# maikmerten/hmp3

Measured on AMD Instinct MI355X. Metric: batched stereo 44.1kHz frames/sec (whole node), CBR-128, higher is better.
Workload: dtype f32; 1 GPU; batch=1024 stereo 44.1kHz streams x 256 frames per step per GPU, CBR-128, long blocks only, int16 PCM resident in HBM; streams_per_gpu=1024, parallelism=streams sharded over 1 GPU(s), no collective

## Files before the change

### hmp3_amd/csrc/hx_alloc.hip

```cpp
#include "hx_dev.h"

#ifndef HX_LSF
#define HX_LSF 0
#endif
#ifndef HX_A1
#define HX_A1 0
#endif
#ifndef HX_SLIM
#define HX_SLIM 0
#endif
#if HX_SLIM && HX_A1
#error "the low-footprint layout is built for the second-generation allocator only"
#endif
#define HX_WAVES (HX_SLIM ? 3 : 2)
#define HX_PERSIST HX_SLIM
#define HX_RATE_SPEED (!HX_SLIM)
#define HX_OPAQUE_LANE HX_SLIM
#define HX_SEEK_FORCEINLINE HX_SLIM
#define HX_LUCKY_K (HX_SLIM ? 6 : 12)
#define GMIN_OFFSET 70
#define PART23 4021
#define NB 22

struct AllocPrm {
    unsigned char head[4];
    int remainder, divisor, main_framebytes, sf_bit_max, AveTargetBits;
    int ms_flag, hf_flag, vbr_flag;
    int ivbr_min, ivbr_max, vbr_main_framebytes[16], vbr_pool_target;
    int fbmin, fbmax;
    int initialMNR, test1;
    int nsf[2], nsf2[2], nsf3[2], nbmax[2], nbmax2[2], nbmax3[2];
    float rnBand_l[22];
    int nsfs, nbmax_s;
    struct { int npart; } psyS;
    int nchan, side_bytes;
    int is_flag, dual, npart_l;
    int oflags;
    int run_w;
};

static_assert(sizeof(HxGr) == 96, "the frame loop copies the four HxGr of a frame as 96 words");
struct alignas(16) Outbox {
    HxSegOut seg[2];
    HxGr gr[2][2];
    int scfsi[2], mdb, part;
    unsigned sidew[10];
    unsigned char head[4];
    HxFrameOut frm;
    HxSlot slot;
    int opos, frm_index, slot_index;
    int ring_p0;
    int has_frame;
};

#if HX_SLIM
typedef short ix_t;
typedef short sgs_t;
typedef signed char sfo_t;
typedef short btab_t;
#else
typedef int ix_t;
typedef int sgs_t;
typedef int sfo_t;
typedef int btab_t;
#endif

struct FrameState {
    int padcount; unsigned main_tot, main_sent, mf_tot;
    int main_bytes; unsigned side_p0, side_p1, tot_frames_out, tot_bytes_out; int ave_tot;
    int opos, slot_lo, slot_hi;
    int pad, byte_pool, byte_max, byte_min, bytesout, pk_first;
};

struct alignas(16) AllocLds {
    float xr[2][576];
    float x34[2][576];
    float term[2][576];
#if !HX_SLIM
    int ix[2][576];
    unsigned char signx[2][576];
    alignas(16) HxBandPrep band_next;
#else
    unsigned long long sgnbits[2][9];
    ix_t ixsink;
#endif
    unsigned char band_of_pair[288];
    unsigned short lane_run[64];
    unsigned char band_last[24];
    float look_ix43[256];
#if !HX_SLIM
    float look_gain[128], look_34igain[128];
    int mblog[256];
    float pow34_exp[256];
    int logsub[84];
#else
    float gain4[4], igain16[16];
    unsigned short mblog[256];
    short logsub[84];
#endif
    float pow34_a[16], pow34_b[16], quant_off[32];
    unsigned char huff_len[1408];
    unsigned char sband_of_line[192];
    btab_t nBand_s[16], startBand_s[16], logcbw_s[16];
    unsigned char quada_len[16];
    btab_t nBand[NB], startBand[24], logcbw[NB], taper[NB];
    int NTadjust[2][NB];
    union {
        struct {
            int snr[2][NB], Noise0[2][NB], Noise[2][NB], NT[2][NB];
            int gzero[2][NB], gmin[2][NB], gsf[2][NB], sf[2][NB], active[2][NB];
            int ixmax[2][NB], ix10xmax[2][NB], up[2][NB], lo[2][NB], geval[2][NB], maskmb[2][NB];
            float xsxx[2][NB], x34max[2][NB];
            float gig[2][NB];
            alignas(8) float2 gpair[2][NB];
            int lucky[HX_LUCKY_K][2][13];
            unsigned short llist[HX_LUCKY_K * 26 + 4];
        };
        struct {
            int a_pad[17][2][NB];
            float a_sig[2][NB], a_smask[2][NB], a_mask[2][NB], a_noise[2][NB];
            int a_lastGsf[2][NB];
        };
        struct {
            int s_snr[2][3][16], s_Noise0[2][3][16], s_Noise[2][3][16], s_NT[2][3][16];
            sgs_t s_gzero[2][3][16], s_gmin[2][3][16], s_gsf[2][3][16], s_sf[2][3][16], s_active[2][3][16];
            int s_ixmax[2][3][16], s_geval[3][16], s_tmpn[3][16], s_maskmb[2][3][16];
            float s_xsxx[2][3][16], s_x34max[2][3][16];
            int s_G[2][3], s_GG[2], s_subgain[2][3];
        };
    };
    int G[2], preemp[2], scale[2], huff_bits[2];
    int hs_table[2][4], hs_cbreg[2][3], hs_nbig[2], hs_nquads[2], hs_bits[2];
    int MNR, PoolFraction, call_count;
    int a_calls, a_bitadjust[2];
    float a_running, a_ave, a_alpha;
    int hf_quant, hf_quant_stereo[2], gsf_hf, gsf_hf_stereo[2];
    int sf_save[2][21];
    int scfsi[2];
    int nchan, block_type, maxBits, maxTargetBits, minTargetBits, PoolBits, TargetBits, deltaMNR, activeBands;
    int tmp[8];
    int tmpn[2][NB];
    unsigned int sidew[10];
    HxGr gr[2][2];
    sfo_t sfout[2][2][NB];
    sfo_t sfs[2][3][12];
    AllocPrm P;
    FrameState fs;
    int tabpk[32];
    unsigned long long candpk[19];
    unsigned short r_mf[32];
    int r_off[32];
#if !HX_SLIM
    float dump[64];
#endif
    Outbox ob[2];
    const double *pow43;
    int *big_counter;
    int nstrict;
#if !HX_SLIM
    int nlucky[3];
#endif
    int cur_s;
    alignas(16) int cmdw[4];
    alignas(4) unsigned char gflag[HX_SLIM ? 64 : 256];
#ifdef HX_PROFILE
    unsigned prof[HX_PROF_WORDS];
#endif
};

#if !HX_SLIM
// ... 88 lines not shown
    const unsigned seg = (u >> 19) & 15;
    const int e = (int) ((u >> 23) & 255), k = 3 * (e - 127);
    float ex = ldexpf(L.gain4[k & 3], k >> 2);
    if (e == 0) ex = 0.0f;
    if (e == 255) ex = hx_bits2f(0x7F800000u);
    return (m * L.pow34_b[seg] + L.pow34_a[seg]) * ex;
}
#else
__device__ __forceinline__ float pow34(const AllocLds &L, float x) { return hx_pow34(L.pow34_a, L.pow34_b, L.pow34_exp, x); }
#endif

__device__ __forceinline__ int logsubber(const AllocLds &L, int n1, int n2)
{
    int k = (n1 - n2) >> 4;
    if (k > 83) k = 83;
    return n1 + L.logsub[k];
}

__device__ __forceinline__ int drop_guard(int noise0, int nt)
{
    int tsnr = noise0 - nt;
    if (tsnr < 300) { tsnr = 187 + ((3 * tsnr) >> 3) - tsnr; nt -= tsnr; }
    return nt;
}

__device__ __forceinline__ int pretab(int i)
{
    return (i < 11 || i > 20) ? 0 : (i < 15 ? 1 : (i < 17 ? 2 : (i < 20 ? 3 : 2)));
}
__device__ __forceinline__ int sf_limit_hi(int scale, int pre, int i)
{
    int base = (i < 11) ? (scale ? 62 : 31) : (scale ? 30 : 15);
    if (pre) base += (scale ? 4 : 2) * pretab(i);
    return base;
}
__device__ __forceinline__ int sf_limit_lo(int scale, int pre, int i) { return pre ? (scale ? 4 : 2) * pretab(i) : 0; }
__device__ __forceinline__ int sf_upper(int scale, int pre, int i)
{
    int base = (i < 11) ? (scale ? 60 : 30) : (scale ? 28 : 14);
    if (pre) base += (scale ? 4 : 2) * pretab(i);
    return base;
}

__device__ __forceinline__ float noise_term(const AllocLds &L, float igain, float gain, float x34, float x, bool *fast)
{
    float tmp = (igain * x34 + (0.0f - 0.0946f));
    const int qx = (int) (tmp + copysignf(0.5f, tmp));
    *fast = (qx >= 0 && qx < 256);
    const float xhat = gain * L.look_ix43[*fast ? qx : 0];
    tmp = x - xhat;
    return tmp * tmp;
}
__device__ __noinline__ double pow43_beyond(int qx) { return pow((double) qx, (4.0 / 3.0)); }
__device__ __forceinline__ float noise_xhat_big(const AllocLds &L, int qx, double pw_tab, float gain)
{
    double pw = pw_tab;
    if (qx >= HX_POW43_N) pw = pow43_beyond(qx);
    return (float) (gain * pw);
}

__device__ __forceinline__ float noise_term_fast(const AllocLds &L, float igain, float gain, float x34, float x)
{
    float tmp = (igain * x34 + (0.0f - 0.0946f));
    const unsigned qx = (unsigned) (int) (tmp + 0.5f);
    const float xhat = gain * L.look_ix43[min(qx, 255u)];
    tmp = x - xhat;
    return tmp * tmp;
}
__device__ __forceinline__ bool noise_band_needs_pow(float igain, float x34max)
{
    const float tmp = (igain * x34max + (0.0f - 0.0946f));
    return (int) (tmp + copysignf(0.5f, tmp)) >= 256;
}

#define RUNW_MAX 10
struct SweepRegs { float x34[RUNW_MAX], xr[RUNW_MAX]; };
struct LaneRun { int start, cnt, d, band; };

__device__ __forceinline__ LaneRun lane_run(const AllocLds &L)
{
    HX_LANE_DECL;
    const unsigned r = L.lane_run[LANE];
    LaneRun q;
    q.start = (int) (r & 511u) << 1; q.cnt = (int) ((r >> 9) & 7u) << 1; q.d = (int) (r >> 12);
    q.band = L.band_of_pair[r & 511u];
    return q;
}

__device__ __forceinline__ void sweep_load(const AllocLds &L, SweepRegs &R, const LaneRun &q, int ch)
{
#pragma unroll
    for (int k = 0; k < RUNW_MAX; k += 2) {
        const int j = min(q.start + k, 576 - 2);
        float2 a = *reinterpret_cast<const float2 *>(&L.x34[ch][j]);
        float2 b = *reinterpret_cast<const float2 *>(&L.xr[ch][j]);
        if (k >= q.cnt) { a = make_float2(0.0f, 0.0f); b = a; }
        R.x34[k] = a.x; R.x34[k + 1] = a.y; R.xr[k] = b.x; R.xr[k + 1] = b.y;
    }
}

__device__ __forceinline__ float sweep_run(const AllocLds &L, const SweepRegs &R, const LaneRun &q, int ch)
{
    const float2 gp = L.gpair[ch][q.band];
    float t[RUNW_MAX];
#pragma unroll
    for (int k = 0; k < RUNW_MAX; k++) t[k] = noise_term_fast(L, gp.x, gp.y, R.x34[k], R.xr[k]);
    return (((t[0] + t[1]) + (t[2] + t[3])) + ((t[4] + t[5]) + (t[6] + t[7]))) + (t[8] + t[9]);
}

__device__ __noinline__ float sweep_run_stored(AllocLds &L, int ch, int W, int count)
{
    HX_LANE_DECL;
    if (count && LANE == 0) atomicAdd(L.big_counter, 1);
    const LaneRun q = lane_run(L);
    const float2 gp = L.gpair[ch][q.band];
    float acc = 0.0f;
#pragma unroll 1
    for (int k = 0; k < W; k += 2) {
        float t[2], xr[2];
        int qx[2];
        const float2 a = *reinterpret_cast<const float2 *>(&L.x34[ch][q.start + k]);
        const float2 b = *reinterpret_cast<const float2 *>(&L.xr[ch][q.start + k]);
        const bool in = k < q.cnt;
        const float x34[2] = {in ? a.x : 0.0f, in ? a.y : 0.0f};
        xr[0] = in ? b.x : 0.0f; xr[1] = in ? b.y : 0.0f;
#pragma unroll
        for (int e = 0; e < 2; e++) {
            const float tmp = (gp.x * x34[e] + (0.0f - 0.0946f));
            qx[e] = (int) (tmp + copysignf(0.5f, tmp));
            t[e] = noise_term_fast(L, gp.x, gp.y, x34[e], xr[e]);
        }
        if (__any(qx[0] >= 256 || qx[1] >= 256)) {
            double pw[2];
#pragma unroll
            for (int e = 0; e < 2; e++) pw[e] = L.pow43[min(max(qx[e], 0), HX_POW43_N - 1)];
#pragma unroll
            for (int e = 0; e < 2; e++)
                if (qx[e] >= 256) { const float d = xr[e] - noise_xhat_big(L, qx[e], pw[e], gp.y); t[e] = d * d; }
        }
        if (in) *reinterpret_cast<float2 *>(&L.term[ch][q.start + k]) = make_float2(t[0], t[1]);
        acc += (t[0] + t[1]);
    }
    return acc;
}

__device__ __noinline__ float sweep_sum_strict(AllocLds &L, int ch, int W, int have_terms, bool need, int sbeg, int n, float fast)
{
    HX_LANE_DECL;
    if (!have_terms) (void) sweep_run_stored(L, ch, W, 0);
    HX_WAVE_SYNC();
    if (LANE == 0) atomicAdd(&L.nstrict, 1);
    float sxx = fast;
    if (need) sxx = band_sum(&L.term[ch][sbeg], n, 0.0f);
    return sxx;
}

__device__ __forceinline__ int noise_sweep(AllocLds &L, const SweepRegs &R, const LaneRun &q, int W, int ch, int g, float ig_g, float gn_g, float x34max, int logcbw, int sbeg, int send, float du, int last4)
{
    HX_LANE_DECL;
    bool bslow = false;
    PROF_T0();
    if (LANE < NB) {
        const float ig = (g >= 0) ? ig_g : -1.0f;
        L.gpair[ch][LANE] = make_float2(ig, (g >= 0) ? gn_g : 0.0f);
        if (g >= 0) bslow = noise_band_needs_pow(ig, x34max);
    }
    HX_WAVE_SYNC();
    PROF_ACC(HX_PROF_SWEEP_PUBLISH);
// ... 394 lines not shown
        g0 = L.gzero[ch][i] - 4;
        s = min(L.sf[ch][i] - sdelta, L.up[ch][i]);
        s0 = L.lo[ch][i];
        nt = L.NT[ch][i];
        mode = 1;
        if (!(s >= s0) || (GG - s) >= g0) mode = 2;
    }
    while (__any(mode == 1)) {
        PROF_CNT(HX_PROF_N_LUCKY);
        PROF_T0();
        int nc = 0;
        if (mode == 1) {
            const int sh = 1 + L.scale[ch];
            nc = min(K, min(((s - s0) >> sh) + 1, (g0 - GG + s + sdelta - 1) >> sh));
        }
        if (i < NB) { L.geval[ch][i] = (mode == 1) ? GG - s : -1; L.tmpn[ch][i] = nc; }
        unsigned short *list = L.llist;
        const int incl = hx_wave_scan(nc), total = __builtin_amdgcn_readlane(incl, 63);
#pragma unroll
        for (int c = 0; c < HX_LUCKY_K; c++) if (c < nc) list[incl - nc + c] = (c << 8) | (ch << 7) | i;
        HX_WAVE_SYNC();
        const int ncmax = hx_wave_max(nc);
#if !HX_SLIM
        npass++; reach = max(reach, ncmax);
#endif
        const bool bslow = mode == 1 && noise_band_needs_pow(LK_IGAIN(GG - s), L.x34max[ch][i]);
        PROF_ACC(HX_PROF_LUCKY_SETUP);
        const bool two = p->nchan == 2;
        const int big = __any(bslow) ? 1 : 0;
        if (two) { if (LANE == 0) L.cmdw[3] = big; HELPER_POST2(HCMD_LUCKY, nl, ncmax); }
        lucky_dispatch(L, nl, ncmax, tf, 0, big);
        if (two) HELPER_JOIN();
        else lucky_dispatch(L, nl, ncmax, tf, 1, big);
        HX_WAVE_SYNC();
        PROF_ACC(HX_PROF_LUCKY_TERMS);
        for (int u = LANE; u < total; u += 64) {
            const int e = list[u], c = e >> 8, cc = (e >> 7) & 1, b = e & 31;
            float sxx = band_sum(tf + c * 2 * nl + cc * nl + L.startBand[b], L.nBand[b], 0.0f);
            L.lucky[c][cc][b] = MBLOG(1.0e-12f + sxx) - L.logcbw[b];
        }
        HX_WAVE_SYNC();
        PROF_ACC(HX_PROF_LUCKY_SUMS);
        {
            int best = 0;
            bool hit = false;
#pragma unroll
            for (int h = 0; h < HX_LUCKY_K; h += 6) {
                if (h == 0 || ncmax > h) {
                    int nz[6];
#pragma unroll
                    for (int c = 0; c < 6; c++) nz[c] = L.lucky[h + c][ch][min(i, 12)];
#pragma unroll
                    for (int c = 0; c < 6; c++)
                        if (h + c < nc && nz[c] <= nt) { best = nz[c]; smin = s - (h + c) * sdelta; hit = true; }
                }
            }
            if (hit) L.Noise[ch][i] = best;
            if (mode == 1) {
                s -= nc * sdelta;
                if (!(s >= s0) || (GG - s) >= g0) mode = 2;
            }
        }
        HX_WAVE_SYNC();
        PROF_ACC(HX_PROF_LUCKY_REPLAY);
    }
    if (mode == 2) {
        L.sf[ch][i] = smin;
        L.gsf[ch][i] = max(GG - smin, 0);
    }
#if !HX_SLIM
    if (reach * 2 * nl > 1152) {
        const int end = reach * 2 * nl - 1152;
        for (int j = p->nbmax[0] + LANE; j < min(end, 576); j += 64) IX(0)[j] = 0;
        for (int j = p->nbmax[1] + LANE; j < end - 576; j += 64) IX(1)[j] = 0;
    }
    if (npass && LANE == 0) { L.nlucky[0] += 1; L.nlucky[1] += npass; L.nlucky[2] += (reach > 6); }
#endif
    HX_WAVE_SYNC();
}

__device__ __forceinline__ void quant_lines(AllocLds &L, const AllocPrm *p, int opt, int c)
{
    HX_LANE_DECL;
    const int nl = p->nbmax[c];
#if HX_SLIM
    const int nfill = (opt & 2) ? nl : 576;
#endif
    const bool tab = (opt & 1) != 0;
    int q[9], b[9];
#pragma unroll
    for (int k = 0; k < 9; k++) b[k] = BAND_OF_LINE(LANE + 64 * k);
#pragma unroll
    for (int k = 0; k < 9; k++) {
        const int j = LANE + 64 * k;
        const float igain = L.gig[c][b[k]];
        const float t = igain * L.x34[c][j] + (tab ? (0.5f - 0.4375f) : (0.5f - 0.0946f));
        const float off = L.quant_off[max(min((int) t, 31), 0)];
        q[k] = (int) (t - (tab ? off : 0.0f));
    }
#pragma unroll
    for (int k = 0; k < 9; k++) {
        const int j = LANE + 64 * k;
#if HX_SLIM
        const int qq = (j < nl) ? q[k] : 0;
        *((j < nfill) ? &IX(c)[j] : &L.ixsink) = (ix_t) qq;
        if (qq > 0) atomicMax(&L.ixmax[c][b[k]], qq);
#else
        if (j < nl) {
            IX(c)[j] = q[k];
            if (q[k] > 0) atomicMax(&L.ixmax[c][b[k]], q[k]);
        }
#endif
    }
}

__device__ void do_quant(AllocLds &L, const AllocPrm *p, int opt)
{
    HX_LANE_DECL;
    const int ch = LANE >> 5, i = LANE & 31;
    if (i < NB) {
        L.ixmax[ch][i] = (i < p->nsf[ch]) ? 0 : L.ixmax[ch][i];
        L.gig[ch][i] = LK_IGAIN(L.gsf[ch][i] & 127);
    }
    HX_WAVE_SYNC();
    const bool two = p->nbmax[1] > 0;
    if (two) HELPER_POST(HCMD_QUANT, opt);
    quant_lines(L, p, opt, 0);
    if (two) HELPER_JOIN();
    HX_WAVE_SYNC();
}

struct Cand { int n, t0, t1, t2, t3, tmax; };

__device__ __forceinline__ Cand mk_cand(int n, int t0, int t1, int t2, int t3, int tmax)
{
    Cand c; c.n = n; c.t0 = t0; c.t1 = t1; c.t2 = t2; c.t3 = t3; c.tmax = tmax;
    return c;
}

__device__ __forceinline__ Cand candidates_chain(int rmax)
{
    if (rmax <= 0) return mk_cand(0, 0, 0, 0, 0, 0);
    if (rmax == 1) return mk_cand(2, 1, 3, 0, 0, 1);
    if (rmax == 2) return mk_cand(2, 2, 3, 0, 0, 2);
    if (rmax == 3) return mk_cand(2, 5, 6, 0, 0, 3);
    if (rmax <= 5) return mk_cand(4, 7, 8, 9, 12, 5);
    if (rmax <= 7) return mk_cand(4, 10, 11, 12, 15, 7);
    if (rmax <= 15) return mk_cand(2, 13, 15, 0, 0, 15);
    if (rmax == 16) return mk_cand(2, 16, 24, 0, 0, 16);
    if (rmax <= 18) return mk_cand(2, 17, 24, 0, 0, 18);
    if (rmax <= 22) return mk_cand(2, 18, 24, 0, 0, 22);
    if (rmax <= 30) return mk_cand(2, 19, 24, 0, 0, 30);
    if (rmax <= 46) return mk_cand(2, 25, 20, 0, 0, 46);
    if (rmax <= 78) return mk_cand(2, 20, 26, 0, 0, 78);
    if (rmax <= 142) return mk_cand(2, 27, 21, 0, 0, 142);
    if (rmax <= 270) return mk_cand(2, 21, 28, 0, 0, 270);
    if (rmax <= 526) return mk_cand(2, 29, 22, 0, 0, 526);
    if (rmax <= 1038) return mk_cand(2, 22, 30, 0, 0, 1038);
    if (rmax <= 2062) return mk_cand(2, 30, 23, 0, 0, 2062);
    return mk_cand(2, 31, 23, 0, 0, 8206);
}

__device__ __forceinline__ int cand_class(int rmax)
{
    if (rmax <= 3) return max(rmax, 0);
    if (rmax <= 15) return rmax <= 5 ? 4 : (rmax <= 7 ? 5 : 6);
    return min(7 + (31 - __clz(rmax - 15)), 18);
}
__device__ __forceinline__ int cand_class_rep(int c)
{
    return c <= 3 ? c : (c == 4 ? 4 : (c == 5 ? 6 : (c == 6 ? 8 : 15 + (1 << (c - 7)))));
}
__device__ __forceinline__ unsigned long long cand_pack(const Cand &c)
{
    return (unsigned long long) (c.n | (c.t0 << 3) | (c.t1 << 8) | (c.t2 << 13) | (c.t3 << 18)) | ((unsigned long long) c.tmax << 23);
}
__device__ __forceinline__ Cand candidates(const AllocLds &L, int rmax)
{
    const unsigned long long pk = L.candpk[cand_class(rmax)];
    const unsigned lo = (unsigned) pk;
    return mk_cand(lo & 7, (lo >> 3) & 31, (lo >> 8) & 31, (lo >> 13) & 31, (lo >> 18) & 31, (int) (pk >> 23));
}

__device__ __forceinline__ int tab_pack(const AllocLds &L, int t) { return L.tabpk[t]; }
__device__ __forceinline__ int pair_len_p(const AllocLds &L, int pk, int x, int y)
{
    const int off = pk & 0xFFF, dim = (pk >> 12) & 0xFF, lin = pk >> 20;
    const int cx = min(x, 15), cy = min(y, 15);
    int n = L.huff_len[off + cx * dim + cy];
    n += (x >= 15 ? lin : 0) + (y >= 15 ? lin : 0);
    return n + (x != 0) + (y != 0);
}

__device__ __forceinline__ int pair_len(const AllocLds &L, int t, int x, int y) { return pair_len_p(L, tab_pack(L, t), x, y); }

__device__ __forceinline__ void acc_pair(const AllocLds &L, const Cand &c, int x, int y, int &p01, int &p23)
{
    if (c.n == 0) return;
    p01 += pair_len(L, c.t0, x, y) | (pair_len(L, c.t1, x, y) << 16);
    if (c.n == 4) p23 += pair_len(L, c.t2, x, y) | (pair_len(L, c.t3, x, y) << 16);
}

__device__ __forceinline__ int pick_table(const Cand &c, int p01, int p23, int live, int *bits)
{
    const int b0 = p01 & 0xFFFF, b1 = (p01 >> 16) & 0xFFFF, b2 = p23 & 0xFFFF, b3 = (p23 >> 16) & 0xFFFF;
    int best = 0, t = c.t0;
// ... 116 lines not shown
            for (int k = 0; k < 5; k++) {
                const int j = 2 * (LANE + 64 * k);
                const int pa = (j < n0) ? qa0 : (j < n1 ? qa1 : qa2), pb = (j < n0) ? qb0 : (j < n1 ? qb1 : qb2);
                acc[k] = pair_len_p(L, pa, xy[k].x, xy[k].y) | (pair_len_p(L, pb, xy[k].x, xy[k].y) << 16);
            }
#pragma unroll
            for (int k = 0; k < 5; k++) {
                const int j = 2 * (LANE + 64 * k);
                const int rn = (j < n0) ? c0.n : (j < n1 ? c1.n : c2.n);
                const int v = (j < nbig && rn == 4) ? acc[k] : 0;
                r0b += (j < n0) ? v : 0;
                r1b += (j >= n0 && j < n1) ? v : 0;
                r2b += (j >= n1) ? v : 0;
            }
        }
    }
    PROF_ACC(HX_PROF_CNT_PAIRS);
    int qa = 0, qb = 0;
    {
        int2 qv[3][2];
#pragma unroll
        for (int k = 0; k < 3; k++) {
            const int q = min(LANE + 64 * k, max(nquads - 1, 0));
#if HX_SLIM
            const uint2 w2 = *reinterpret_cast<const uint2 *>(ix + nbig + 4 * q);
            qv[k][0] = make_int2((int) (w2.x & 0xFFFFu), (int) (w2.x >> 16)); qv[k][1] = make_int2((int) (w2.y & 0xFFFFu), (int) (w2.y >> 16));
#else
            const int2 *v2 = reinterpret_cast<const int2 *>(ix + nbig + 4 * q);
            qv[k][0] = v2[0]; qv[k][1] = v2[1];
#endif
        }
#pragma unroll
        for (int k = 0; k < 3; k++) {
            const int v0 = qv[k][0].x, v1 = qv[k][0].y, v2 = qv[k][1].x, v3 = qv[k][1].y;
            const int pop = v0 + v1 + v2 + v3;
            const int la = L.quada_len[((v0 << 3) + (v1 << 2) + (v2 << 1) + v3) & 15] + pop;
            const bool ok = LANE + 64 * k < nquads;
            qa += ok ? la : 0;
            qb += ok ? 4 + pop : 0;
        }
    }
    PROF_ACC(HX_PROF_CNT_QUADS);
    r0a = hx_wave_sum(r0a); r2a = hx_wave_sum(r2a);
    r0b = hx_wave_sum(r0b); r2b = hx_wave_sum(r2b);
    r1a = hx_wave_sum(r1a); r1b = hx_wave_sum(r1b);
    int bits = 0;
    const int tab0 = pick_table(c0, r0a, r0b, n0 > 0, &bits);
    int tab1 = pick_table(c1, r1a, r1b, (n1 - n0 > 0) && bt == 0, &bits);
    const int tab2 = pick_table(c2, r2a, r2b, nbig - n1 > 0, &bits);
    if (bt != 0) tab1 = tab2;
    {
        const int q = hx_wave_sum(qa | (qb << 16));
        qa = q & 0xFFFF;
        qb = (q >> 16) & 0xFFFF;
    }
    int qidx = 0;
    if (nquads > 0) { if (qa < qb) { bits += qa; qidx = 0; } else { bits += qb; qidx = 1; } }
    if (LANE == 0) {
        L.hs_table[ch][0] = tab0; L.hs_table[ch][1] = tab1; L.hs_table[ch][2] = tab2; L.hs_table[ch][3] = qidx;
        L.hs_cbreg[ch][0] = cb0; L.hs_cbreg[ch][1] = cb1; L.hs_cbreg[ch][2] = cb2;
        L.hs_nbig[ch] = nbig; L.hs_nquads[ch] = nquads; L.hs_bits[ch] = bits;
        L.huff_bits[ch] = bits;
    }
    PROF_ACC(HX_PROF_CNT_REDUCE);
    return bits;
}

__device__ int count_bits(AllocLds &L, const AllocPrm *p, const int *ncb)
{
    HX_LANE_DECL;
    PROF_CNT(HX_PROF_N_COUNTS);
    const bool two = p->nchan == 2;
    if (two) HELPER_POST(HCMD_COUNT_BITS, ncb[1]);
    int bits = count_bits_ch(L, p, 0, ncb[0]);
    if (two) { HELPER_JOIN(); bits += L.hs_bits[1]; }
    HX_WAVE_SYNC();
    return bits;
}

__device__ int quant_count_bits(AllocLds &L, const AllocPrm *p, int opt, int zero21, const int *ncb)
{
    HX_LANE_DECL;
    const int ch = LANE >> 5, i = LANE & 31;
    if (i < NB) {
        L.ixmax[ch][i] = (i < p->nsf[ch]) ? 0 : L.ixmax[ch][i];
        L.gig[ch][i] = LK_IGAIN(L.gsf[ch][i] & 127);
    }
    HX_WAVE_SYNC();
    PROF_CNT(HX_PROF_N_COUNTS);
    const bool two = p->nchan == 2;
    PROF_T0();
    if (two) HELPER_POST2(HCMD_QUANT_COUNT, opt, ncb[1]);
    PROF_ACC(HX_PROF_QC_POST);
    quant_lines(L, p, opt, 0);
    HX_WAVE_SYNC();
    PROF_ACC(HX_PROF_QC_QUANT);
    if (zero21) { if (LANE == 0) L.ixmax[0][21] = 0; HX_WAVE_SYNC(); }
    int bits = count_bits_ch(L, p, 0, ncb[0]);
    PROF_T1();
    if (two) { HELPER_JOIN(); bits += L.hs_bits[1]; }
    HX_WAVE_SYNC();
    PROF_ACC(HX_PROF_QC_JOIN);
    return bits;
}

#include "hx_alloc2.inc"
#include "hx_alloc_short.inc"
#if HX_A1
#include "hx_alloc1.inc"
#endif
#include "hx_alloc3.inc"
```

### hmp3_amd/csrc/hx_alloc3.inc

```

#define COLD(field) (((const __attribute__((address_space(4))) AllocArgs *) __builtin_amdgcn_kernarg_segment_ptr())->field)
#define RFL(x) __builtin_amdgcn_readfirstlane(x)

__device__ __noinline__ void emit_packet(AllocLds &L, const AllocPrm *p, unsigned char *q, int *nbytes, int pad, int ms, int raw_bytes, int hdr, int lsf_igr)
{
    HX_LANE_DECL;
    if (LANE < 4) {
        unsigned char h = p->head[LANE];
        if (LANE == 2 && pad) h |= 2;
        if (LANE == 3) h = (unsigned char) ((h & 0xCF) | ((ms + ms + (HX_A1 ? p->is_flag : 0)) << 4));
        q[LANE] = h;
    }
    if (lsf_igr >= 0) pack_side_lsf(L, p, q + 4, lsf_igr, 0);
    else pack_side(L, p, q + 4, 0);
    if (LANE == 0) *nbytes = hdr + raw_bytes;
}

template <int LSF>
__device__ __forceinline__ int pack_sf_any(AllocLds &L, int pos, int igr, int ch, int bt, int use_scfsi, int not_null, int *sc, unsigned short *sfdst)
{
    HX_LANE_DECL;
    *sc = 0;
    int field = 0;
    if (LSF) {
// ... 189 lines not shown
        L.xr[0][j] = o0; L.xr[1][j] = o1;
    }
}

__device__ __forceinline__ void x34_from_coded(AllocLds &L, int ms)
{
    HX_LANE_DECL;
    const int nl0 = ms ? L.P.nbmax2[0] : L.P.nbmax3[0], nl1 = ms ? L.P.nbmax2[1] : L.P.nbmax3[1];
    float a[9], b[9];
#pragma unroll
    for (int k = 0; k < 9; k++) { a[k] = L.xr[0][LANE + 64 * k]; b[k] = L.xr[1][LANE + 64 * k]; }
#pragma unroll
    for (int k = 0; k < 9; k++) {
        const int j = LANE + 64 * k;
        L.x34[0][j] = (j < nl0) ? pow34(L, a[k]) : 0.0f;
        L.x34[1][j] = (j < nl1) ? pow34(L, b[k]) : 0.0f;
    }
}

template <int LSF>
__device__ __forceinline__ void helper_serve(const AllocArgs &a, AllocLds &L)
{
    for (;;) {
        HX_LANE_DECL;
        WG_BARRIER();
        const int4 order = *reinterpret_cast<const int4 *>(&L.cmdw[0]);
        const int cmd = order.x;
        if (cmd == HCMD_SEEK) seek_actual_ch(L, &L.P, 1);
        else if (cmd == HCMD_COUNT_BITS) count_bits_ch(L, &L.P, 1, order.y);
        else if (cmd == HCMD_LUCKY) lucky_dispatch(L, order.y, order.z, &L.term[0][0], 1, order.w);
        else if (cmd == HCMD_QUANT) quant_lines(L, &L.P, order.y, 1);
        else if (cmd == HCMD_QUANT_COUNT) { quant_lines(L, &L.P, order.y, 1); HX_WAVE_SYNC(); count_bits_ch(L, &L.P, 1, order.z); }
        else if (cmd == HCMD_ISF2) isf2_ch(L, &L.P, 1);
        else if (cmd == HCMD_FETCH) {
            const int s = L.cur_s;
            int nbt = 2, nms = 0;
            if (order.y >= 0) {
                granule_fetch(L, a, (long long) s * a.NG + order.y);
                nbt = a.bt[(long long) s * a.NG + order.y]; nms = a.msflag[(long long) s * a.NG + order.y];
            }
            const int gl = order.z, gf = (gl >= 0) ? gl - 1 : ((order.y < 0) ? order.w : -1);
            LinesRegs lr0 = {}, lr1 = {};
            OutRegs orr = {};
            const int two = L.P.nchan == 2;
            const int gbt = order.w & 255;
            if (gl >= 0) { lines_gather(L, (order.w >> 8) & 1, 0, gbt, lr0); if (two) lines_gather(L, (order.w >> 9) & 1, 1, gbt, lr1); }
            if (gf >= 0) outbox_gather(L, gf, orr);
            asm volatile("s_waitcnt vmcnt(0) lgkmcnt(0)" ::: "memory");
            const bool long_gr = !HX_A1 && nbt != 2;
            if (long_gr) {
                xr_to_coded(L, nms);
                if (!two) x34_from_coded(L, nms);
                asm volatile("s_waitcnt lgkmcnt(0)" ::: "memory");
            }
            WG_BARRIER();
            if (gl >= 0) {
                const long long unit = (long long) s * a.NG + gl;
                lines_store(a, unit, 0, gbt, lr0);
                if (two) lines_store(a, unit, 1, gbt, lr1);
            }
            if (gf >= 0) outbox_store<LSF>(L, a, s, gf, orr);
            if (long_gr && two) { x34_from_coded(L, nms); asm volatile("s_waitcnt lgkmcnt(0)" ::: "memory"); }
            continue;
        }
        else if (cmd == HCMD_EXIT) return;
        WG_BARRIER();
    }
}

__device__ __forceinline__ void stage_stream(const AllocArgs &a, AllocLds &L, const HxStream *ss, const HxParams *gp, const HxGlobalTabs *gt)
{
    HX_LANE_DECL;
#if HX_SLIM
    for (int i = LANE; i < 256; i += 64) { L.look_ix43[i] = gp->look_ix43[i]; L.mblog[i] = (unsigned short) (gt->mblog[i] + 38227); }
    if (LANE < 4) L.gain4[LANE] = gp->look_gain[8 + LANE];
    if (LANE < 16) L.igain16[LANE] = gp->look_34igain[8 + LANE];
    if (LANE < 18) L.sgnbits[LANE / 9][LANE % 9] = 0;
#else
    for (int i = LANE; i < 256; i += 64) { L.look_ix43[i] = gp->look_ix43[i]; L.mblog[i] = gt->mblog[i]; L.pow34_exp[i] = gt->pow34_exp[i]; }
    for (int i = LANE; i < 128; i += 64) { L.look_gain[i] = gp->look_gain[i]; L.look_34igain[i] = gp->look_34igain[i]; }
#endif
    for (int i = LANE; i < 1408; i += 64) L.huff_len[i] = gt->huff_len[i];
    for (int i = LANE; i < 288; i += 64) L.band_of_pair[i] = gp->band_of_line[2 * i];
    L.lane_run[LANE] = gp->lane_run[LANE];
    if (LANE < 24) L.band_last[LANE] = gp->band_last_lane[LANE];
    for (int i = LANE; i < 192; i += 64) L.sband_of_line[i] = gp->sband_of_line[i];
    if (LANE < 16) {
        L.nBand_s[LANE] = (LANE < 13) ? gp->nBand_s[LANE] : 0;
        L.startBand_s[LANE] = (LANE < 14) ? gp->startBand_s[LANE] : 192;
        L.logcbw_s[LANE] = gp->look_log_cbwmb_s[LANE];
    }
    for (int i = LANE; i < 84; i += 64) L.logsub[i] = (HX_SLIM ? (short) gt->logsub[i] : gt->logsub[i]);
    if (LANE < 32) L.quant_off[LANE] = gt->quant_off[LANE];
    if (LANE < 32) {
        const int dim = (LANE >= 16) ? 16 : gt->huff_dim[LANE], lin = (LANE >= 16) ? gt->huff_lin[LANE] : 0;
        L.tabpk[LANE] = gt->huff_off[LANE] | (dim << 12) | (lin << 20);
    }
    if (LANE < 19) L.candpk[LANE] = cand_pack(candidates_chain(cand_class_rep(LANE)));
    if (LANE < 16) {
        L.pow34_a[LANE] = gt->pow34_a[LANE]; L.pow34_b[LANE] = gt->pow34_b[LANE];
        L.quada_len[LANE] = gt->quada_len[LANE];
    }
    if (LANE < 24) L.startBand[LANE] = gp->startBand_l[LANE];
    if (LANE < NB) { L.nBand[LANE] = gp->nBand_l[LANE]; L.logcbw[LANE] = gp->look_log_cbwmb[LANE]; L.taper[LANE] = gp->taperNT[LANE]; }
#if !HX_SLIM
    for (int i = LANE; i < 2 * 576; i += 64) { IX(0)[i] = 0; (&L.signx[0][0])[i] = 0; }
#endif
    if (LANE < 44) {
        int c = LANE / 22, b = LANE % 22;
        L.NTadjust[c][b] = ss->NTadjust[c][b];
        L.ixmax[c][b] = 0; L.sf[c][b] = 0; L.active[c][b] = 0; L.gsf[c][b] = 0; L.gzero[c][b] = 0; L.gmin[c][b] = 0;
        L.x34max[c][b] = 0.0f; L.Noise[c][b] = 0; L.Noise0[c][b] = 0; L.NT[c][b] = 0; L.geval[c][b] = -1;
        L.up[c][b] = 0; L.lo[c][b] = 0;
    }
    if (LANE < 42) L.sf_save[LANE / 21][LANE % 21] = ss->sf_save[LANE / 21][LANE % 21];
    if (LANE == 0) { L.pow43 = gt->pow43; L.big_counter = COLD(done_counter) + HX_CNT_BIG_SWEEPS; L.nstrict = 0; }
#if !HX_SLIM
    if (LANE < 3) L.nlucky[LANE] = 0;
#endif
    if (LANE < 4) L.P.head[LANE] = gp->head[LANE];
    if (LANE < 16) L.P.vbr_main_framebytes[LANE] = gp->vbr_main_framebytes[LANE];
    if (LANE < 22) L.P.rnBand_l[LANE] = gp->rnBand_l[LANE];
    if (LANE < 2) {
        const bool on = LANE < gp->nchan;
        L.P.nsf[LANE] = on ? gp->nsf[LANE] : 0; L.P.nsf2[LANE] = on ? gp->nsf2[LANE] : 0; L.P.nsf3[LANE] = on ? gp->nsf3[LANE] : 0;
        L.P.nbmax[LANE] = on ? gp->nbmax[LANE] : 0; L.P.nbmax2[LANE] = on ? gp->nbmax2[LANE] : 0; L.P.nbmax3[LANE] = on ? gp->nbmax3[LANE] : 0;
    }
    if (LANE == 0) {
        L.P.remainder = gp->remainder; L.P.divisor = gp->divisor; L.P.main_framebytes = gp->main_framebytes;
        L.P.sf_bit_max = gp->sf_bit_max; L.P.AveTargetBits = gp->AveTargetBits;
        L.P.ms_flag = gp->ms_flag; L.P.hf_flag = gp->hf_flag; L.P.vbr_flag = gp->vbr_flag;
        L.P.ivbr_min = gp->ivbr_min; L.P.ivbr_max = gp->ivbr_max; L.P.vbr_pool_target = gp->vbr_pool_target;
        L.P.fbmin = gp->vbr_main_framebytes[gp->ivbr_min & 15]; L.P.fbmax = gp->vbr_main_framebytes[gp->ivbr_max & 15];
        L.P.initialMNR = gp->initialMNR; L.P.test1 = gp->test1;
        L.P.nsfs = gp->nsfs; L.P.nbmax_s = gp->nbmax_s; L.P.psyS.npart = gp->psyS.npart;
        L.P.nchan = gp->nchan; L.P.side_bytes = gp->side_bytes;
        L.P.is_flag = gp->is_flag; L.P.dual = gp->alloc1 && gp->h_mode == 2; L.P.npart_l = gp->psyL.npart;
        L.P.oflags = (a.packet ? 1 : 0) | (a.dbg ? 2 : 0) | (a.frame_stats ? 4 : 0) | (a.strict_sums ? 8 : 0);
        L.P.run_w = gp->run_w;
    }
#if HX_A1
    for (int i = LANE; i < 256; i += 64) {
        (&L.term[0][0])[i] = gp->a1_f_ix[i]; (&L.term[0][0])[256 + i] = gp->a1_f_ixmax[i];
        (&L.term[0][0])[512 + i] = gp->a1_f_big_ix[i]; (&L.term[0][0])[768 + i] = gp->a1_f_big_ixmax[i];
    }
    if (LANE < 42) L.gsf[LANE / 21][LANE % 21] = ss->a1_gsf[LANE / 21][LANE % 21];
    if (LANE == 0) {
        L.a_calls = ss->a1_call_count; L.a_bitadjust[0] = ss->a1_bitadjust[0]; L.a_bitadjust[1] = ss->a1_bitadjust[1];
        L.a_running = ss->a1_running_a; L.a_ave = ss->a1_ave_alpha; L.a_alpha = ss->a1_alpha;
    }
#endif
    if (LANE == 0) {
        L.MNR = ss->MNR; L.PoolFraction = ss->PoolFraction; L.call_count = ss->call_count;
        L.hf_quant = 0; L.hf_quant_stereo[0] = L.hf_quant_stereo[1] = 0; L.gsf_hf = -1;
        L.gsf_hf_stereo[0] = L.gsf_hf_stereo[1] = -1;
        L.scfsi[0] = L.scfsi[1] = 0;
        for (int g = 0; g < 2; g++) for (int c = 0; c < 2; c++) {
            HxGr z = {};
            L.gr[g][c] = z;
            for (int k = 0; k < 3; k++) L.gr[g][c].subblock_gain[k] = ss->gr_subblock_gain[g][c][k];
        }
    }
#ifdef HX_PROFILE
    L.prof[LANE] = 0;
    if (LANE == 0) L.prof[HX_PROF_TOTAL] = (unsigned) clock64();
#endif
    HX_WAVE_SYNC();
// ... 494 lines not shown
```

### hmp3_amd/csrc/hx_dev.h

```cpp
#pragma once
#include <hip/hip_runtime.h>
#include "hx_types.h"

#define HX_WAVE 64

#define HX_WAVE_SYNC() do { asm volatile("" ::: "memory"); __builtin_amdgcn_wave_barrier(); } while (0)
#define HX_LDS __attribute__((address_space(3)))
#define HX_GLB __attribute__((address_space(1)))

__device__ __forceinline__ float hx_bits2f(unsigned u) { return __uint_as_float(u); }
__device__ __forceinline__ unsigned hx_f2bits(float f) { return __float_as_uint(f); }

__device__ __forceinline__ int hx_mblog(const int *tab, float x)
{
    unsigned u = hx_f2bits(x);
    return tab[(u >> 15) & 255] + 301 * (int) (u >> 23);
}

__device__ __forceinline__ int hx_mblog16(const unsigned short *tab, float x)
{
    unsigned u = hx_f2bits(x);
    return (int) tab[(u >> 15) & 255] + 301 * (int) (u >> 23) - 38227;
}

// ... 1 lines not shown
{
    float t = lo[(unsigned) x & 0xff] * hi[((unsigned) x & 0xff00) >> 8];
    if (x > 32000) return 1.0E32f;
    if (x < -32000) return 1.0E-32f;
    return t;
}

__device__ __forceinline__ int hx_round(float x) { return (int) (x + copysignf(0.5f, x)); }

#define HX_DPP(old, src, ctrl, rmask) __builtin_amdgcn_update_dpp((old), (src), (ctrl), (rmask), 0xf, false)
#define HX_SCAN_ROWS(v, ident, OP)                                                    \
    v = OP(v, HX_DPP(ident, v, 0x111, 0xf));                            \
    v = OP(v, HX_DPP(ident, v, 0x112, 0xf));                            \
    v = OP(v, HX_DPP(ident, v, 0x114, 0xf));                            \
    v = OP(v, HX_DPP(ident, v, 0x118, 0xf));                            \
    v = OP(v, HX_DPP(ident, v, 0x142, 0xa));
#define HX_SCAN_WAVE(v, ident, OP)                                                    \
    HX_SCAN_ROWS(v, ident, OP)                                                        \
    v = OP(v, HX_DPP(ident, v, 0x143, 0xc));
#define HX_OP_ADD(a, b) ((a) + (b))
#define HX_OP_MAX(a, b) max((a), (b))
#define HX_OP_OR(a, b) ((a) | (b))

__device__ __forceinline__ int hx_wave_sum(int v)
{
    HX_SCAN_WAVE(v, 0, HX_OP_ADD)
    return __builtin_amdgcn_readlane(v, 63);
}
__device__ __forceinline__ int hx_wave_max(int v)
{
    HX_SCAN_WAVE(v, (int) 0x80000000, HX_OP_MAX)
    return __builtin_amdgcn_readlane(v, 63);
}
__device__ __forceinline__ int hx_wave_or(int v)
{
    HX_SCAN_WAVE(v, 0, HX_OP_OR)
    return __builtin_amdgcn_readlane(v, 63);
}
__device__ __forceinline__ int hx_wave_scan(int v)
{
    HX_SCAN_WAVE(v, 0, HX_OP_ADD)
    return v;
}
__device__ __forceinline__ int hx_half_sum(int v)
{
    HX_SCAN_ROWS(v, 0, HX_OP_ADD)
    const int lo = __builtin_amdgcn_readlane(v, 31), hi = __builtin_amdgcn_readlane(v, 63);
    return (threadIdx.x & 32) ? hi : lo;
}
__device__ __forceinline__ int hx_half_max(int v)
{
    HX_SCAN_ROWS(v, (int) 0x80000000, HX_OP_MAX)
    const int lo = __builtin_amdgcn_readlane(v, 31), hi = __builtin_amdgcn_readlane(v, 63);
    return (threadIdx.x & 32) ? hi : lo;
}
__device__ __forceinline__ int hx_half_or(int v)
{
    HX_SCAN_ROWS(v, 0, HX_OP_OR)
    const int lo = __builtin_amdgcn_readlane(v, 31), hi = __builtin_amdgcn_readlane(v, 63);
    return (threadIdx.x & 32) ? hi : lo;
}

__device__ __forceinline__ float hx_pow34(const float *a, const float *b, const float *ex, float x)
{
    unsigned u = hx_f2bits(x);
    float m = hx_bits2f((u & 0x7FFFFFu) | (127u << 23));
    unsigned seg = (u >> 19) & 15, e = (u >> 23) & 255;
    return (m * b[seg] + a[seg]) * ex[e];
}

#define HX_DPPF(v, ctrl, rmask) __int_as_float(__builtin_amdgcn_update_dpp(0, __float_as_int(v), (ctrl), (rmask), 0xf, false))
__device__ __forceinline__ float hx_seg_scan(float v, int d, int lane)
{
    float t;
    t = HX_DPPF(v, 0x111, 0xf); v += (d >= 1) ? t : 0.0f;
    t = HX_DPPF(v, 0x112, 0xf); v += (d >= 2) ? t : 0.0f;
    t = HX_DPPF(v, 0x114, 0xf); v += (d >= 4) ? t : 0.0f;
    t = HX_DPPF(v, 0x118, 0xf); v += (d >= 8) ? t : 0.0f;
    const bool cross = d > (lane & 15);
    t = HX_DPPF(v, 0x142, 0xa); v += cross ? t : 0.0f;
    t = HX_DPPF(v, 0x143, 0x4); v += cross ? t : 0.0f;
    return v;
}
__device__ __forceinline__ float hx_lane_read(int src4, float v) { return __int_as_float(__builtin_amdgcn_ds_bpermute(src4, __float_as_int(v))); }
__device__ __forceinline__ float hx_cert_delta(int n, int W) { return (float) (n + W + 16) * 5.9604644775390625e-08f; }
__device__ __forceinline__ bool hx_cert_mblog(float t, float du)
{
    const float e = t * du;
    return (hx_f2bits(1.0e-12f + (t - e)) >> 15) == (hx_f2bits(1.0e-12f + (t + e)) >> 15);
}
__device__ __forceinline__ bool hx_cert_mblog_ratio(float x, float q, float du)
{
    const float ex = x * du, eq = q * du;
    return (hx_f2bits((x - ex) / (q + eq)) >> 15) == (hx_f2bits((x + ex) / (q - eq)) >> 15);
}

__device__ __forceinline__ float band_sum(const float *t, int n, float acc)
{
    const float2 *t2 = reinterpret_cast<const float2 *>(t);
    const int m = n >> 1;
    int j = 0;
    if (m >= 8) {
        float2 c[8], nx[8];
#pragma unroll
        for (int k = 0; k < 8; k++) c[k] = t2[k];
        for (j = 8; j + 8 <= m; j += 8) {
#pragma unroll
            for (int k = 0; k < 8; k++) nx[k] = t2[j + k];
#pragma unroll
            for (int k = 0; k < 8; k++) { acc += c[k].x; acc += c[k].y; }
#pragma unroll
            for (int k = 0; k < 8; k++) c[k] = nx[k];
        }
#pragma unroll
        for (int k = 0; k < 8; k++) { acc += c[k].x; acc += c[k].y; }
    }
    if (j + 4 <= m) {
        float2 a = t2[j], b = t2[j + 1], c = t2[j + 2], d = t2[j + 3];
        acc += a.x; acc += a.y; acc += b.x; acc += b.y;
        acc += c.x; acc += c.y; acc += d.x; acc += d.y;
        j += 4;
    }
    if (j + 2 <= m) {
        float2 a = t2[j], b = t2[j + 1];
        acc += a.x; acc += a.y; acc += b.x; acc += b.y;
        j += 2;
    }
    if (j < m) { float2 a = t2[j]; acc += a.x; acc += a.y; }
    return acc;
}
__device__ __forceinline__ void band_sum2(const float *t, const float *u, int n, float *s0, float *s1)
{
    const float2 *t2 = reinterpret_cast<const float2 *>(t), *u2 = reinterpret_cast<const float2 *>(u);
    const int m = n >> 1;
    float a0 = 0.0f, a1 = 0.0f;
    int j = 0;
    if (m >= 8) {
        float2 c[8], d[8], nc[8], nd[8];
#pragma unroll
        for (int k = 0; k < 8; k++) { c[k] = t2[k]; d[k] = u2[k]; }
        for (j = 8; j + 8 <= m; j += 8) {
#pragma unroll
            for (int k = 0; k < 8; k++) { nc[k] = t2[j + k]; nd[k] = u2[j + k]; }
#pragma unroll
            for (int k = 0; k < 8; k++) { a0 += c[k].x; a1 += d[k].x; a0 += c[k].y; a1 += d[k].y; }
#pragma unroll
            for (int k = 0; k < 8; k++) { c[k] = nc[k]; d[k] = nd[k]; }
        }
#pragma unroll
        for (int k = 0; k < 8; k++) { a0 += c[k].x; a1 += d[k].x; a0 += c[k].y; a1 += d[k].y; }
    }
    if (j + 4 <= m) {
        float2 c[4], d[4];
#pragma unroll
        for (int k = 0; k < 4; k++) { c[k] = t2[j + k]; d[k] = u2[j + k]; }
#pragma unroll
        for (int k = 0; k < 4; k++) { a0 += c[k].x; a1 += d[k].x; a0 += c[k].y; a1 += d[k].y; }
        j += 4;
    }
    if (j + 2 <= m) {
        float2 c0 = t2[j], c1 = t2[j + 1], d0 = u2[j], d1 = u2[j + 1];
        a0 += c0.x; a1 += d0.x; a0 += c0.y; a1 += d0.y;
        a0 += c1.x; a1 += d1.x; a0 += c1.y; a1 += d1.y;
        j += 2;
    }
    if (j < m) { float2 c0 = t2[j], d0 = u2[j]; a0 += c0.x; a1 += d0.x; a0 += c0.y; a1 += d0.y; }
// ... 5 lines not shown
```

Baseline: 18.03 million frames/s.

## Quantize lines by per-lane band runs with DPP segmented max instead of atomics

Quantization is restructured so each lane processes a contiguous run of lines from the precomputed lane_run table, and the band number is now packed into that table's upper bits. Per-band maxima come from a segmented DPP max-scan with one writer per band, replacing per-element LDS atomicMax and the separate zeroing of ixmax. Stores become packed 2-element writes, and the slim layout's sink slot is dropped in favour of an explicit tail-zero loop. This removes LDS atomic contention and per-line band lookups, at the cost of extra scan instructions and assumptions about how runs map onto bands.

```diff
diff --git a/hmp3_amd/csrc/hx_alloc.hip b/hmp3_amd/csrc/hx_alloc.hip
--- a/hmp3_amd/csrc/hx_alloc.hip
+++ b/hmp3_amd/csrc/hx_alloc.hip
@@ -82,10 +82,9 @@
     alignas(16) HxBandPrep band_next;
 #else
     unsigned long long sgnbits[2][9];
-    ix_t ixsink;
 #endif
     unsigned char band_of_pair[288];
-    unsigned short lane_run[64];
+    unsigned lane_run[64];
     unsigned char band_last[24];
     float look_ix43[256];
 #if !HX_SLIM
@@ -340,8 +339,8 @@
     HX_LANE_DECL;
     const unsigned r = L.lane_run[LANE];
     LaneRun q;
-    q.start = (int) (r & 511u) << 1; q.cnt = (int) ((r >> 9) & 7u) << 1; q.d = (int) (r >> 12);
-    q.band = L.band_of_pair[r & 511u];
+    q.start = (int) (r & 511u) << 1; q.cnt = (int) ((r >> 9) & 7u) << 1; q.d = (int) ((r >> 12) & 15u);
+    q.band = (int) (r >> 16);
     return q;
 }
 
@@ -902,46 +901,48 @@
 __device__ __forceinline__ void quant_lines(AllocLds &L, const AllocPrm *p, int opt, int c)
 {
     HX_LANE_DECL;
-    const int nl = p->nbmax[c];
+    const bool tab = (opt & 1) != 0;
+    const LaneRun q = lane_run(L);
+    const unsigned nxt = L.lane_run[min(LANE + 1, 63)];
+    const float igain = L.gig[c][q.band];
+    const bool coded = q.band < p->nsf[c];
+    const int ncoded = coded ? q.cnt : 0;
+    float2 x[RUNW_MAX / 2];
+#pragma unroll
+    for (int k = 0; k < RUNW_MAX; k += 2) x[k >> 1] = *reinterpret_cast<const float2 *>(&L.x34[c][min(q.start + k, 576 - 2)]);
+    int qv[RUNW_MAX], m = 0;
+#pragma unroll
+    for (int k = 0; k < RUNW_MAX; k++) {
+        const float t = igain * ((k & 1) ? x[k >> 1].y : x[k >> 1].x) + (tab ? (0.5f - 0.4375f) : (0.5f - 0.0946f));
+        const float off = L.quant_off[max(min((int) t, 31), 0)];
+        const int v = (int) (t - (tab ? off : 0.0f));
+        qv[k] = (k < ncoded) ? v : 0;
+        m = max(m, qv[k]);
+    }
+    const bool last = q.cnt > 0 && (LANE == 63 || ((nxt >> 12) & 15u) == 0);
+    m = hx_seg_scan_max(m, q.d, LANE);
+    if (last && coded) L.ixmax[c][q.band] = m;
 #if HX_SLIM
-    const int nfill = (opt & 2) ? nl : 576;
-#endif
-    const bool tab = (opt & 1) != 0;
-    int q[9], b[9];
-#pragma unroll
-    for (int k = 0; k < 9; k++) b[k] = BAND_OF_LINE(LANE + 64 * k);
-#pragma unroll
-    for (int k = 0; k < 9; k++) {
-        const int j = LANE + 64 * k;
-        const float igain = L.gig[c][b[k]];
-        const float t = igain * L.x34[c][j] + (tab ? (0.5f - 0.4375f) : (0.5f - 0.0946f));
-        const float off = L.quant_off[max(min((int) t, 31), 0)];
-        q[k] = (int) (t - (tab ? off : 0.0f));
-    }
-#pragma unroll
-    for (int k = 0; k < 9; k++) {
-        const int j = LANE + 64 * k;
-#if HX_SLIM
-        const int qq = (j < nl) ? q[k] : 0;
-        *((j < nfill) ? &IX(c)[j] : &L.ixsink) = (ix_t) qq;
-        if (qq > 0) atomicMax(&L.ixmax[c][b[k]], qq);
+    const bool fill = !(opt & 2);
+    const int nwritten = fill ? q.cnt : ncoded;
+#pragma unroll
+    for (int k = 0; k < RUNW_MAX; k += 2)
+        if (k < nwritten)
+            *reinterpret_cast<unsigned *>(IX(c) + q.start + k) = ((unsigned) qv[k] & 0xFFFFu) | ((unsigned) qv[k + 1] << 16);
+    if (fill)
+        for (int j = max(p->nbmax[0], p->nbmax[1]) + 2 * LANE; j < 576; j += 128) *reinterpret_cast<unsigned *>(IX(c) + j) = 0u;
 #else
-        if (j < nl) {
-            IX(c)[j] = q[k];
-            if (q[k] > 0) atomicMax(&L.ixmax[c][b[k]], q[k]);
-        }
-#endif
-    }
+#pragma unroll
+    for (int k = 0; k < RUNW_MAX; k += 2)
+        if (k < ncoded) *reinterpret_cast<int2 *>(IX(c) + q.start + k) = make_int2(qv[k], qv[k + 1]);
+#endif
 }
 
 __device__ void do_quant(AllocLds &L, const AllocPrm *p, int opt)
 {
     HX_LANE_DECL;
     const int ch = LANE >> 5, i = LANE & 31;
-    if (i < NB) {
-        L.ixmax[ch][i] = (i < p->nsf[ch]) ? 0 : L.ixmax[ch][i];
-        L.gig[ch][i] = LK_IGAIN(L.gsf[ch][i] & 127);
-    }
+    if (i < NB) L.gig[ch][i] = LK_IGAIN(L.gsf[ch][i] & 127);
     HX_WAVE_SYNC();
     const bool two = p->nbmax[1] > 0;
     if (two) HELPER_POST(HCMD_QUANT, opt);
@@ -1224,10 +1225,7 @@
 {
     HX_LANE_DECL;
     const int ch = LANE >> 5, i = LANE & 31;
-    if (i < NB) {
-        L.ixmax[ch][i] = (i < p->nsf[ch]) ? 0 : L.ixmax[ch][i];
-        L.gig[ch][i] = LK_IGAIN(L.gsf[ch][i] & 127);
-    }
+    if (i < NB) L.gig[ch][i] = LK_IGAIN(L.gsf[ch][i] & 127);
     HX_WAVE_SYNC();
     PROF_CNT(HX_PROF_N_COUNTS);
     const bool two = p->nchan == 2;
diff --git a/hmp3_amd/csrc/hx_alloc3.inc b/hmp3_amd/csrc/hx_alloc3.inc
--- a/hmp3_amd/csrc/hx_alloc3.inc
+++ b/hmp3_amd/csrc/hx_alloc3.inc
@@ -295,7 +295,7 @@
 #endif
     for (int i = LANE; i < 1408; i += 64) L.huff_len[i] = gt->huff_len[i];
     for (int i = LANE; i < 288; i += 64) L.band_of_pair[i] = gp->band_of_line[2 * i];
-    L.lane_run[LANE] = gp->lane_run[LANE];
+    { const unsigned r = gp->lane_run[LANE]; L.lane_run[LANE] = r | ((unsigned) gp->band_of_line[2 * (r & 511u)] << 16); }
     if (LANE < 24) L.band_last[LANE] = gp->band_last_lane[LANE];
     for (int i = LANE; i < 192; i += 64) L.sband_of_line[i] = gp->sband_of_line[i];
     if (LANE < 16) {
diff --git a/hmp3_amd/csrc/hx_dev.h b/hmp3_amd/csrc/hx_dev.h
--- a/hmp3_amd/csrc/hx_dev.h
+++ b/hmp3_amd/csrc/hx_dev.h
@@ -107,6 +107,18 @@
     t = HX_DPPF(v, 0x143, 0x4); v += cross ? t : 0.0f;
     return v;
 }
+__device__ __forceinline__ int hx_seg_scan_max(int v, int d, int lane)
+{
+    int t;
+    t = HX_DPP(0, v, 0x111, 0xf); v = max(v, (d >= 1) ? t : 0);
+    t = HX_DPP(0, v, 0x112, 0xf); v = max(v, (d >= 2) ? t : 0);
+    t = HX_DPP(0, v, 0x114, 0xf); v = max(v, (d >= 4) ? t : 0);
+    t = HX_DPP(0, v, 0x118, 0xf); v = max(v, (d >= 8) ? t : 0);
+    const bool cross = d > (lane & 15);
+    t = HX_DPP(0, v, 0x142, 0xa); v = max(v, cross ? t : 0);
+    t = HX_DPP(0, v, 0x143, 0x4); v = max(v, cross ? t : 0);
+    return v;
+}
 __device__ __forceinline__ float hx_lane_read(int src4, float v) { return __int_as_float(__builtin_amdgcn_ds_bpermute(src4, __float_as_int(v))); }
 __device__ __forceinline__ float hx_cert_delta(int n, int W) { return (float) (n + W + 16) * 5.9604644775390625e-08f; }
 __device__ __forceinline__ bool hx_cert_mblog(float t, float du)
```

New measurement: 18.16 million frames/s (median of 6 runs). Within noise of the previous version (+0.7%).
